# Datou/Datou-gomoku-muzero

Measured on AMD Instinct MI355X. Metric: self-play moves/sec (15x15, 400 sims), higher is better.
Workload: dtype fp16

## Files before the change

### datou-gomoku-muzero_amd/csrc/gmz_conv.hip

```cpp
#include <initializer_list>
#include <type_traits>

#include "gmz_common.h"

#include <hip/hip_bf16.h>
#include <hip/hip_fp16.h>

namespace gmz {
namespace {

typedef _Float16 f16x8_t __attribute__((ext_vector_type(8)));
typedef __bf16 b16x8_t __attribute__((ext_vector_type(8)));
typedef float f32x4_t __attribute__((ext_vector_type(4)));
typedef uint16_t u16x4_t __attribute__((ext_vector_type(4)));

#ifndef GMZ_CONV_RD
#define GMZ_CONV_RD 3
#endif
constexpr int CC = 128;
constexpr int CKSTEPS = 36;
constexpr int FRAG_BYTES = 294912;

__device__ __forceinline__ int csigma16(int j) { return j < 8 ? (j ^ 4) : j; }

template <int H>
struct CImg {
  static constexpr int HP = H + 2, PS = 272, RS = HP * PS - 32;
  static constexpr int BYTES = ((HP - 1) * RS + HP * PS + 255) / 256 * 256;
  static constexpr int RUN = (H - 1) * PS + 256;
  static constexpr int RUN_DMA = (RUN + 1023) / 1024;
};

template <typename T> struct Mfma;
template <> struct Mfma<__half> {
  typedef f16x8_t V;
  static __device__ __forceinline__ f32x4_t run(V a, V b, f32x4_t c) {
    return __builtin_amdgcn_mfma_f32_16x16x32_f16(a, b, c, 0, 0, 0);
  }
  static __device__ __forceinline__ uint16_t bits(float f) { return __builtin_bit_cast(uint16_t, (_Float16)f); }
  static __device__ __forceinline__ float value(uint16_t u) { return (float)__builtin_bit_cast(_Float16, u); }
};
template <> struct Mfma<__hip_bfloat16> {
  typedef b16x8_t V;
  static __device__ __forceinline__ f32x4_t run(V a, V b, f32x4_t c) {
    return __builtin_amdgcn_mfma_f32_16x16x32_bf16(a, b, c, 0, 0, 0);
  }
  static __device__ __forceinline__ uint16_t bits(float f) { return __builtin_bit_cast(uint16_t, (__bf16)f); }
  static __device__ __forceinline__ float value(uint16_t u) { return __uint_as_float(((uint32_t)u) << 16); }
};

__device__ __forceinline__ int chunk_of(int ks, int g) { return 2 * ks + ((g & 1) * 8 + (g >> 1)); }

template <typename T>
__global__ void __launch_bounds__(256) k_pack_conv(const float *__restrict__ w, long s0, long s1, long s2, long s3,
                                                   int transpose, uint16_t *__restrict__ out) {
  const int i = blockIdx.x * 256 + threadIdx.x;
  if (i >= CKSTEPS * 8 * 64) return;
  const int l = i & 63, nt = (i >> 6) & 7, st = i >> 9, t = st >> 2, ks = st & 3;
  const int n = nt * 16 + (l & 15);
  u16x4_t lo, hi;
#pragma unroll
  for (int j = 0; j < 8; ++j) {
    const int c = chunk_of(ks, l >> 4) * 8 + j;
    const int o = transpose ? c : n, ci = transpose ? n : c, tt = transpose ? 8 - t : t;
    const float v = w[o * s0 + ci * s1 + (tt / 3) * s2 + (tt % 3) * s3];
    const uint16_t b = Mfma<T>::bits(v);
    if (j < 4) lo[j] = b;
    else hi[j - 4] = b;
  }
  uint4 r;
  r.x = (uint32_t)lo[0] | ((uint32_t)lo[1] << 16);
  r.y = (uint32_t)lo[2] | ((uint32_t)lo[3] << 16);
  r.z = (uint32_t)hi[0] | ((uint32_t)hi[1] << 16);
  r.w = (uint32_t)hi[2] | ((uint32_t)hi[3] << 16);
  *(uint4 *)(out + (size_t)i * 8) = r;
}

struct PackJob {
  const float *w;
  long long s0, s1, s2, s3;
  uint16_t *out;
  int transpose, pad;
};

template <typename T>
__global__ void __launch_bounds__(256) k_pack_many(const PackJob *__restrict__ jobs) {
  const PackJob j = jobs[blockIdx.y];
  const int i = blockIdx.x * 256 + threadIdx.x;
  if (i >= CKSTEPS * 8 * 64) return;
  const int l = i & 63, nt = (i >> 6) & 7, st = i >> 9, t = st >> 2, ks = st & 3;
  const int n = nt * 16 + (l & 15);
  u16x4_t lo, hi;
#pragma unroll
  for (int e = 0; e < 8; ++e) {
    const int c = chunk_of(ks, l >> 4) * 8 + e;
    const int o = j.transpose ? c : n, ci = j.transpose ? n : c, tt = j.transpose ? 8 - t : t;
    const uint16_t b = Mfma<T>::bits(j.w[o * j.s0 + ci * j.s1 + (tt / 3) * j.s2 + (tt % 3) * j.s3]);
    if (e < 4) lo[e] = b;
    else hi[e - 4] = b;
  }
  uint4 r;
  r.x = (uint32_t)lo[0] | ((uint32_t)lo[1] << 16);
  r.y = (uint32_t)lo[2] | ((uint32_t)lo[3] << 16);
  r.z = (uint32_t)hi[0] | ((uint32_t)hi[1] << 16);
  r.w = (uint32_t)hi[2] | ((uint32_t)hi[3] << 16);
  *(uint4 *)(j.out + (size_t)i * 8) = r;
}

struct BnBwd {
  const uint16_t *x, *y;
  const float *save;
  int relu;
};

struct ActStamp {
  const int32_t *action;
  const float *table;
};

struct BnApply {
  const uint16_t *z, *res;
  const float *gamma, *beta, *save;
  uint16_t *out;
  int relu;
};

template <int... Hs> struct SizeList {};
using ConvSizes = SizeList<6, 9, 15, 19>;

#ifndef GMZ_CONV_PG19
#define GMZ_CONV_PG19 2
#endif
template <int H> struct ConvCfg { static constexpr int PG = 2, WG_PER_CU = 2; static constexpr bool AB = H == 9 || H == 15; };
template <> struct ConvCfg<19> { static constexpr int PG = GMZ_CONV_PG19, WG_PER_CU = 1; static constexpr bool AB = false; };

template <int H, typename T, int PG, bool BWD = false, bool PB = false, bool BNA = false>
__global__ void __launch_bounds__(128 * PG, ConvCfg<H>::WG_PER_CU) k_conv3(const uint16_t *__restrict__ x, const uint16_t *__restrict__ wpk,
                                                  uint16_t *__restrict__ y, int N, const uint8_t *__restrict__ mask,
                                                  double *__restrict__ stats, const uint16_t *__restrict__ addend,
                                                  BnBwd bn, ActStamp as, BnApply ba) {
  using I = CImg<H>;
  using M = Mfma<T>;
  typedef typename M::V V;
  constexpr int A = H * H, NPT = (A + 15) / 16;
  constexpr int NTW = 2, PTW = (NPT + PG - 1) / PG, RD = GMZ_CONV_RD, NW = 2 * PG, NTHR = 64 * NW;
  constexpr int PS = I::PS, RS = I::RS;
  static_assert(CKSTEPS % RD == 0, "ring slots repeat per item");
  constexpr bool REMAP = false;
  constexpr bool LAST_ONE = !REMAP && NPT == PG * (PTW - 1) + 1;
  constexpr unsigned LAST_TAPS = LAST_ONE ? live_taps(H, (NPT - 1) * 16, A) : 0x1ffu;
  static_assert(LAST_TAPS & 1u, "tap 0 of the last tile starts its accumulation");
  __shared__ __attribute__((aligned(16))) uint8_t img[I::BYTES];
  static_assert(I::BYTES >= PG * 64 * 2 * 4, "stats scratch fits in the image");
  static_assert(!PB || !BWD, "per-board statistics: forward sums");
  static_assert(!BNA || (!BWD && !PB), "BatchNorm-apply prologue: the forward with per-workgroup statistics");
  static_assert(NTHR % 16 == 0, "BNA: a thread's chunk of every cell it stages is tid & 15");
  __shared__ float pbred[PB ? PG * 64 * 2 : 1];

  const int tid = threadIdx.x, w = tid >> 6, lane = tid & 63;
  const int nq = w & 1, pg = w >> 1;
  const int g4 = lane >> 4;
  const int cg = (g4 & 1) * 8 + (g4 >> 1);
  const int half0 = (blockIdx.x >> 3) & 1;
  const int b0 = (int)((blockIdx.x >> 4) * 8 + (blockIdx.x & 7));
  const int bstride = (int)(gridDim.x >> 1);
  const int ntile0 = half0 * 4 + nq * NTW;

  {
    constexpr int HP = I::HP, NBORDER = 2 * HP + 2 * H;
    for (int i = tid; i < NBORDER * 16; i += NTHR) {
      const int k = i >> 4, r = k - 2 * HP;
      const int yy = k < HP ? 0 : k < 2 * HP ? HP - 1 : 1 + (r >> 1);
      const int xx = k < HP ? k : k < 2 * HP ? k - HP : (r & 1) * (HP - 1);
      ((uint4 *)(img + yy * RS + xx * PS))[i & 15] = make_uint4(0, 0, 0, 0);
    }
  }

  auto tile_p = [&](int pt) {
    if constexpr (REMAP) {
      const int p = pt < NPT ? remap15(pt, csigma16(lane & 15)) : -1;
      return p < 0 ? A : p;
    }
    const int p = pt * 16 + csigma16(lane & 15);
    return (pt < NPT && p < A) ? p : A;
  };
  int pos[PTW];
#pragma unroll
  for (int i = 0; i < PTW; ++i) {
    const int pt = pg + PG * i, p = tile_p(pt);
    const int pad = REMAP ? 16 * ((remap15_key0(pt) + csigma16(lane & 15)) & 15)
                          : ((A - 1) / H) * RS + ((A - 1) % H) * PS;
    pos[i] = p < A ? (p / H) * RS + (p % H) * PS : ~pad;
  }
  const __amdgpu_buffer_rsrc_t wrsrc = __builtin_amdgcn_make_buffer_rsrc((void *)wpk, (short)0, FRAG_BYTES, 0x00020000);
  const int wvoff = ntile0 * 1024 + lane * 16;
  V ar[RD][NTW];
  auto loadA = [&](int slot, int st) {
    const int soff = (st < CKSTEPS ? st : st - CKSTEPS) * 8192;
#pragma unroll
    for (int nt = 0; nt < NTW; ++nt)
      ar[slot][nt] = __builtin_bit_cast(V, __builtin_amdgcn_raw_buffer_load_b128(wrsrc, wvoff + nt * 1024, soff, 0));
  };
#pragma unroll
  for (int k = 0; k < RD - 1; ++k) loadA(k, k);
  __syncthreads();
  float s1[NTW][4], s2[NTW][4];
#pragma unroll
  for (int nt = 0; nt < NTW; ++nt)
#pragma unroll
    for (int e = 0; e < 4; ++e) s1[nt][e] = s2[nt][e] = 0.f;
  int nvalid = 0;

  auto dma = [&](int bd) {
    const uint8_t *src = (const uint8_t *)(x + (size_t)bd * A * CC);
    for (int j = w; j < H * I::RUN_DMA; j += NW) {
      const int yy = j / I::RUN_DMA, piece = j % I::RUN_DMA;
      const int o = piece * 1024 + lane * 16;
      const int xx = o / PS, ch = (o % PS) >> 4;
      if (o < I::RUN && ch < 16)
        __builtin_amdgcn_global_load_lds((const void *)(src + (yy * H + xx) * 256 + ch * 16),
                                         (__attribute__((address_space(3))) void *)(img + (yy + 1) * RS + PS + piece * 1024),
                                         16, 0, 0);
    }
  };
  auto bn_stage = [&](int bd) {
    int t = tid;
    asm volatile("" : "+v"(t));
    const int bch = t & 15;
    float bmu[8], bsc[8], bsh[8];
#pragma unroll
    for (int j = 0; j < 8; ++j) {
      const int c = bch * 8 + j;
      bmu[j] = ba.save[c];
      bsc[j] = ba.gamma[c] * ba.save[CC + c];
      bsh[j] = ba.beta[c];
    }
    constexpr int NCH = A * 16, NI = (NCH + NTHR - 1) / NTHR, U = 8;
    const size_t base = (size_t)bd * NCH;
    const uint4 *zs = (const uint4 *)ba.z + base;
    const uint4 *rs = ba.res ? (const uint4 *)ba.res + base : nullptr;
    uint4 *os = (uint4 *)ba.out + base;
    const bool mine = (bch >> 3) == half0;
    const uint32_t nz = M::bits(-0.f) * 0x10001u;
    const float lo = ba.relu ? 0.f : -__builtin_inff();
#pragma unroll
    for (int i0 = 0; i0 < NI; i0 += U) {
      uint4 zv[U], rv[U];
#pragma unroll
      for (int u = 0; u < U; ++u) {
        const int i = t + (i0 + u) * NTHR;
        rv[u] = make_uint4(nz, nz, nz, nz);
        if (i0 + u < NI && i < NCH) {
          zv[u] = zs[i];
          if (rs) rv[u] = rs[i];
        }
      }
#pragma unroll
      for (int u = 0; u < U; ++u) {
        const int i = t + (i0 + u) * NTHR;
        if (!(i0 + u < NI && i < NCH)) continue;
        const uint32_t *zw = (const uint32_t *)&zv[u], *rw = (const uint32_t *)&rv[u];
        uint32_t ow[4];
#pragma unroll
        for (int h = 0; h < 4; ++h) {
          uint32_t packed = 0;
#pragma unroll
          for (int e = 0; e < 2; ++e) {
            const int j = 2 * h + e;
            float v = (M::value((uint16_t)(zw[h] >> (16 * e))) - bmu[j]) * bsc[j] + bsh[j];
            v += M::value((uint16_t)(rw[h] >> (16 * e)));
            v = fmaxf(v, lo);
            packed |= (uint32_t)M::bits(v) << (16 * e);
          }
          ow[h] = packed;
        }
        const uint4 o = make_uint4(ow[0], ow[1], ow[2], ow[3]);
        const int p = i >> 4;
        ((uint4 *)(img + (p / H + 1) * RS + (p % H + 1) * PS))[bch] = o;
        if (mine) os[i] = o;
      }
    }
  };
  int mrow = 1;
  if (mask) {
    const int bj = b0 + lane * bstride;
    mrow = bj < N ? (int)mask[bj] : 0;
  }
  for (int b = b0, j = 0; b < N; b += bstride, ++j) {
    if constexpr (BNA) {
      bn_stage(b);
    } else {
      dma(b);
      asm volatile("s_waitcnt vmcnt(0)" ::: "memory");
    }
    __syncthreads();
    const bool counted = stats && (!mask || (j < WAVE ? __builtin_amdgcn_readlane(mrow, j) != 0 : mask[b] != 0));
    nvalid += counted;

    f32x4_t acc[NTW][PTW];
    int bb[PTW];
#pragma unroll
    for (int i = 0; i < PTW; ++i) bb[i] = (pos[i] < 0 ? ~pos[i] : pos[i]) + cg * 16;
    auto kloop = [&](auto ntl_c) {
      constexpr int NTL = decltype(ntl_c)::value;
      V bf[2][NTL];
      constexpr int PGK = NTL == PTW ? 0 : 1;
      auto taps = [&](int i) -> unsigned {
        if constexpr (REMAP) return remap15_taps(PGK + PG * i);
        return (LAST_ONE && NTL == PTW && i == NTL - 1) ? LAST_TAPS : 0x1ffu;
      };
      auto live = [&](int i, int st) { return ((taps(i) >> (st >> 2)) & 1u) != 0; };
      auto first = [&](int i) { return 4 * __builtin_ctz(taps(i)); };
      auto readB = [&](int buf, int st) {
        const int tap = st >> 2, ks = st & 3;
        const int off = (tap / 3) * RS + (tap % 3) * PS + ks * 32;
#pragma unroll
        for (int i = 0; i < NTL; ++i)
          if (live(i, st)) bf[buf][i] = *(const V *)(img + bb[i] + off);
      };
      readB(0, 0);
#pragma unroll
      for (int st = 0; st < CKSTEPS; ++st) {
        loadA((st + RD - 1) % RD, st + RD - 1);
        if (st + 1 < CKSTEPS) readB((st + 1) & 1, st + 1);
        __builtin_amdgcn_sched_barrier(0);
#pragma unroll
        for (int i = 0; i < NTL; ++i)
          if (live(i, st))
#pragma unroll
            for (int nt = 0; nt < NTW; ++nt)
              acc[nt][i] = M::run(ar[st % RD][nt], bf[st & 1][i], st == first(i) ? f32x4_t{0.f, 0.f, 0.f, 0.f} : acc[nt][i]);
        if (st + 1 < CKSTEPS) __builtin_amdgcn_sched_barrier(0);
      }
#pragma unroll
      for (int i = NTL; i < PTW; ++i)
#pragma unroll
        for (int nt = 0; nt < NTW; ++nt) acc[nt][i] = f32x4_t{0.f, 0.f, 0.f, 0.f};
    };
    if constexpr (PTW * PG == NPT) kloop(std::integral_constant<int, PTW>{});
    else if (pg + PG * (PTW - 1) < NPT) kloop(std::integral_constant<int, PTW>{});
    else kloop(std::integral_constant<int, PTW - 1>{});

    uint16_t *dst = y + (size_t)b * A * CC;
    int say = -100, sax = -100;
    if (as.action) {
      const int av = as.action[b];
      say = av / H;
      sax = av - say * H;
    }
    const uint16_t *add = addend ? addend + (size_t)b * A * CC : nullptr;
    float mu[NTW][4], isd[NTW][4];
    if constexpr (BWD) {
#pragma unroll
      for (int nt = 0; nt < NTW; ++nt)
#pragma unroll
        for (int e = 0; e < 4; ++e) {
          const int c = (ntile0 + nt) * 16 + g4 * 4 + e;
          mu[nt][e] = bn.save[c];
          isd[nt][e] = bn.save[CC + c];
        }
    }
#pragma unroll
    for (int i = 0; i < PTW; ++i) {
      const int p = tile_p(pg + PG * i);
      if (p >= A) continue;
#pragma unroll
      for (int nt = 0; nt < NTW; ++nt) {
        const int n0 = (ntile0 + nt) * 16 + g4 * 4;
        u16x4_t o;
        {
          const int ddy = say - p / H + 1, ddx = sax - p % H + 1;
          if (ddy >= 0 && ddy <= 2 && ddx >= 0 && ddx <= 2) {
            const float *tb = as.table + (ddy * 3 + ddx) * CC + n0;
#pragma unroll
            for (int e = 0; e < 4; ++e) acc[nt][i][e] += tb[e];
          }
        }
        if (add) {
          const u16x4_t ad = *(const u16x4_t *)(add + (size_t)p * CC + n0);
#pragma unroll
          for (int e = 0; e < 4; ++e) o[e] = M::bits(acc[nt][i][e] + M::value(ad[e]));
        } else {
#pragma unroll
          for (int e = 0; e < 4; ++e) o[e] = M::bits(acc[nt][i][e]);
        }
        *(u16x4_t *)(dst + (size_t)p * CC + n0) = o;
        if (counted) {
          if constexpr (BWD) {
            const size_t k = ((size_t)b * A + p) * CC + n0;
            const u16x4_t xv = *(const u16x4_t *)(bn.x + k), yv = *(const u16x4_t *)(bn.y + k);
#pragma unroll
            for (int e = 0; e < 4; ++e) {
              float g = M::value(o[e]);
              if (bn.relu && !(M::value(yv[e]) > 0.f)) g = 0.f;
              s1[nt][e] += g;
              s2[nt][e] = fmaf(g, (M::value(xv[e]) - mu[nt][e]) * isd[nt][e], s2[nt][e]);
            }
          } else {
#pragma unroll
            for (int e = 0; e < 4; ++e) {
              const float v = M::value(o[e]);
              s1[nt][e] += v;
              s2[nt][e] = fmaf(v, v, s2[nt][e]);
            }
          }
        }
      }
    }
    if constexpr (PB) {
      if (stats) {
#pragma unroll
        for (int nt = 0; nt < NTW; ++nt)
#pragma unroll
          for (int e = 0; e < 4; ++e)
#pragma unroll
            for (int o = 1; o < 16; o <<= 1) {
              s1[nt][e] += __shfl_xor(s1[nt][e], o, 64);
              s2[nt][e] += __shfl_xor(s2[nt][e], o, 64);
            }
        if ((lane & 15) == 0) {
#pragma unroll
          for (int nt = 0; nt < NTW; ++nt)
#pragma unroll
            for (int e = 0; e < 4; ++e) {
              const int cl = (nq * NTW + nt) * 16 + g4 * 4 + e;
              pbred[(pg * 64 + cl) * 2] = s1[nt][e];
              pbred[(pg * 64 + cl) * 2 + 1] = s2[nt][e];
            }
        }
#pragma unroll
        for (int nt = 0; nt < NTW; ++nt)
#pragma unroll
          for (int e = 0; e < 4; ++e) s1[nt][e] = s2[nt][e] = 0.f;
        __syncthreads();
        if (tid < 64) {
          double a = 0.0, q = 0.0;
#pragma unroll
          for (int g = 0; g < PG; ++g) {
            a += (double)pbred[(g * 64 + tid) * 2];
            q += (double)pbred[(g * 64 + tid) * 2 + 1];
          }
          double *out = stats + ((size_t)(half0 * 64 + tid) * N + b) * 3;
          out[0] = a;
          out[1] = q;
          out[2] = counted ? (double)A : 0.0;
// ... 140 lines not shown
        arl[slot][nt] = __builtin_bit_cast(
            V, __builtin_amdgcn_raw_buffer_load_b128(wrsrc, wvoff + nt * 1024, FRAG_BYTES + st * 8192, 0));
    }
  };
#pragma unroll
  for (int k = 0; k < RD - 1; ++k) loadA(k, k);

  auto stage = [&](int bd, auto lo_c) {
    constexpr bool LO = decltype(lo_c)::value;
    int t = tid;
    asm volatile("" : "+v"(t));
    const int bch = t & 15;
    constexpr int NCH = A * 16, NI = (NCH + NTHR - 1) / NTHR, U = 4;
    const float4 *src = (const float4 *)(x + (size_t)bd * A * CC);
#pragma unroll
    for (int i0 = 0; i0 < NI; i0 += U) {
      float4 va[U], vb[U];
#pragma unroll
      for (int u = 0; u < U; ++u) {
        const int i = t + (i0 + u) * NTHR;
        if (i0 + u < NI && i < NCH) {
          va[u] = src[2 * i];
          vb[u] = src[2 * i + 1];
        }
      }
#pragma unroll
      for (int u = 0; u < U; ++u) {
        const int i = t + (i0 + u) * NTHR;
        if (!(i0 + u < NI && i < NCH)) continue;
        const float f[8] = {va[u].x, va[u].y, va[u].z, va[u].w, vb[u].x, vb[u].y, vb[u].z, vb[u].w};
        uint32_t ow[4];
#pragma unroll
        for (int h = 0; h < 4; ++h) {
          const uint16_t e0 = LO ? split_lo(f[2 * h]) : split_hi(f[2 * h]);
          const uint16_t e1 = LO ? split_lo(f[2 * h + 1]) : split_hi(f[2 * h + 1]);
          ow[h] = (uint32_t)e0 | ((uint32_t)e1 << 16);
        }
        const int p = i >> 4;
        ((uint4 *)(img + (p / H + 1) * RS + (p % H + 1) * PS))[bch] = make_uint4(ow[0], ow[1], ow[2], ow[3]);
      }
    }
  };

  for (int b = b0; b < N; b += bstride) {
    f32x4_t am[NTW][PTW], ac[NTW][PTW];
#pragma unroll
    for (int nt = 0; nt < NTW; ++nt)
#pragma unroll
      for (int i = 0; i < PTW; ++i) am[nt][i] = ac[nt][i] = f32x4_t{0.f, 0.f, 0.f, 0.f};
    auto kloop = [&](auto ntl_c, auto pass_c) {
      constexpr int NTL = decltype(ntl_c)::value, PASS = decltype(pass_c)::value;
      V bf[NTL];
      auto live = [&](int i, int st) {
        const unsigned taps = (LAST_ONE && NTL == PTW && i == NTL - 1) ? LAST_TAPS : 0x1ffu;
        return ((taps >> (st >> 2)) & 1u) != 0;
      };
      auto readB = [&](int i, int st) {
        const int tap = st >> 2, ks = st & 3;
        bf[i] = *(const V *)(img + bb[i] + (tap / 3) * RS + (tap % 3) * PS + ks * 32);
      };
#pragma unroll
      for (int i = 0; i < NTL; ++i) readB(i, 0);
#pragma unroll
      for (int st = 0; st < CKSTEPS; ++st) {
        constexpr int S0 = PASS * CKSTEPS;
        loadA((S0 + st + RD - 1) % RD, S0 + st + RD - 1);
#pragma unroll
        for (int i = 0; i < NTL; ++i) {
          if (live(i, st)) {
#pragma unroll
            for (int nt = 0; nt < NTW; ++nt) {
              if constexpr (PASS == 0) {
                am[nt][i] = M::run(arh[(S0 + st) % RD][nt], bf[i], am[nt][i]);
                ac[nt][i] = M::run(arl[(S0 + st) % RD][nt], bf[i], ac[nt][i]);
              } else {
                ac[nt][i] = M::run(arh[(S0 + st) % RD][nt], bf[i], ac[nt][i]);
              }
            }
          }
          if (st + 1 < CKSTEPS && live(i, st + 1)) readB(i, st + 1);
          __builtin_amdgcn_sched_barrier(0);
        }
      }
    };
    auto pass = [&](auto pass_c) {
      if constexpr (PTW * PG == NPT) kloop(std::integral_constant<int, PTW>{}, pass_c);
      else if (pg + PG * (PTW - 1) < NPT) kloop(std::integral_constant<int, PTW>{}, pass_c);
      else kloop(std::integral_constant<int, PTW - 1>{}, pass_c);
    };
    stage(b, std::false_type{});
    __syncthreads();
    pass(std::integral_constant<int, 0>{});
    __syncthreads();
    stage(b, std::true_type{});
    __syncthreads();
    pass(std::integral_constant<int, 1>{});

    int ln = lane;
    asm volatile("" : "+v"(ln));
    const int eg4 = ln >> 4, ecol = csigma16(ln & 15);
    float *dst = y + (size_t)b * A * CC;
    const float *rsd = bn.res ? bn.res + (size_t)b * A * CC : nullptr;
    float mu[NTW][4], sc[NTW][4], sh[NTW][4];
    if (bn.gamma) {
#pragma unroll
      for (int nt = 0; nt < NTW; ++nt)
#pragma unroll
        for (int e = 0; e < 4; ++e) {
          const int c = (ntile0 + nt) * 16 + eg4 * 4 + e;
          mu[nt][e] = bn.mean[c];
          sc[nt][e] = bn.gamma[c] * (1.0f / sqrtf(bn.var[c] + bn.eps));
          sh[nt][e] = bn.beta[c];
        }
    }
#pragma unroll
    for (int i = 0; i < PTW; ++i) {
      const int pt = pg + PG * i, p = pt * 16 + ecol;
      if (pt >= NPT || p >= A) continue;
#pragma unroll
      for (int nt = 0; nt < NTW; ++nt) {
        const int n0 = (ntile0 + nt) * 16 + eg4 * 4;
        f32x4_t o;
#pragma unroll
        for (int e = 0; e < 4; ++e) o[e] = am[nt][i][e] + ac[nt][i][e] * SPLIT_INV;
        if (bn.gamma) {
          f32x4_t r = {0.f, 0.f, 0.f, 0.f};
          if (rsd) r = *(const f32x4_t *)(rsd + (size_t)p * CC + n0);
#pragma unroll
          for (int e = 0; e < 4; ++e) {
            float v = (o[e] - mu[nt][e]) * sc[nt][e] + sh[nt][e];
            if (rsd) v += r[e];
            o[e] = bn.relu ? fmaxf(v, 0.f) : v;
          }
        }
        *(f32x4_t *)(dst + (size_t)p * CC + n0) = o;
      }
    }
    __syncthreads();
  }
}

typedef short s16x4_t __attribute__((ext_vector_type(4)));

template <int H>
struct WgLds {
  static constexpr int A = H * H, RB = 288, HP = H + 2;
  static constexpr int NB = H > 15 ? 2 : 1, BR = (H + NB - 1) / NB;
  static constexpr int BA = BR * H;
  static constexpr int KS = (BA + 31) / 32, NPOS = KS * 32;
  static constexpr int DY_BYTES = NPOS * RB, X_OFF = DY_BYTES, X_BYTES = (NB == 1 ? HP : BR) * HP * RB;
  static constexpr int BYTES = DY_BYTES + X_BYTES;
  static constexpr int NPD = (BA * RB + 1023) / 1024;
  static constexpr int RUN = (H - 1) * RB + 256, RUN_DMA = (RUN + 1023) / 1024;
};

__device__ __forceinline__ s16x4_t tr_read(const uint8_t *lds_base, int off) {
  return __builtin_amdgcn_ds_read_tr16_b64_v4i16((__attribute__((address_space(3))) s16x4_t *)(
      (__attribute__((address_space(3))) uint8_t *)lds_base + off));
}

constexpr int WG_MAX_SEGS = 8;
struct WgSrc {
  const uint16_t *x[WG_MAX_SEGS];
  const uint16_t *dy[WG_MAX_SEGS];
  int nps;
};

template <int H, typename T>
__global__ void __launch_bounds__(512, 1) k_conv3_wgrad(WgSrc src, int N, int nch, float *__restrict__ part) {
  using L = WgLds<H>;
  using M = Mfma<T>;
  typedef typename M::V V;
  constexpr int A = H * H, KS = L::KS, RB = L::RB, HP = L::HP;
  static_assert(L::BYTES <= 163840, "LDS budget");
  __shared__ __attribute__((aligned(16))) uint8_t smem[L::BYTES];
  uint8_t *xt = smem + L::X_OFF;

  const int tid = threadIdx.x, w = tid >> 6, lane = tid & 63;
  const int xcd = blockIdx.x & 7, slot = blockIdx.x >> 3;
  const int ty = slot % 3, chunk = (slot / 3) * 8 + xcd;
  const int wo = w & 3, wc = w >> 2;
  const int g = lane >> 4, q = (lane >> 2) & 3, pp = lane & 3;
  const int ocol = (wo * 32 + 4 * pp) * 2, ccol = (wc * 64 + 4 * pp) * 2;

  auto zero_cell = [&](uint8_t *cellp, int i) { ((uint4 *)cellp)[i & 15] = make_uint4(0, 0, 0, 0); };
  if constexpr (L::NB == 1) {
    constexpr int NTAIL = L::NPOS - A, NBORDER = 2 * HP + 2 * H;
    for (int i = tid; i < (NTAIL + NBORDER) * 16; i += 512) {
      const int k = i >> 4;
      uint8_t *cellp;
      if (k < NTAIL) {
        cellp = smem + (A + k) * RB;
      } else {
        const int kb = k - NTAIL, r = kb - 2 * HP;
        const int yy = kb < HP ? 0 : kb < 2 * HP ? HP - 1 : 1 + (r >> 1);
        const int xx = kb < HP ? kb : kb < 2 * HP ? kb - HP : (r & 1) * (HP - 1);
        cellp = xt + (yy * HP + xx) * RB;
      }
      ((uint4 *)cellp)[i & 15] = make_uint4(0, 0, 0, 0);
    }
  } else {
    constexpr int NTAIL = L::NPOS - L::BA, NBORDER = 2 * L::BR;
    for (int i = tid; i < (NTAIL + NBORDER) * 16; i += 512) {
      const int k = i >> 4, kb = k - NTAIL;
      zero_cell(k < NTAIL ? smem + (L::BA + k) * RB : xt + ((kb >> 1) * HP + (kb & 1) * (HP - 1)) * RB, i);
    }
  }
  __syncthreads();

  f32x4_t acc[3][2][4];
#pragma unroll
  for (int tx = 0; tx < 3; ++tx)
#pragma unroll
    for (int mt = 0; mt < 2; ++mt)
#pragma unroll
      for (int nt = 0; nt < 4; ++nt) acc[tx][mt][nt] = f32x4_t{0.f, 0.f, 0.f, 0.f};

  for (int b = chunk; b < N; b += nch) {
    const int sg = b / src.nps, lb = b - sg * src.nps;
    const uint8_t *sd = (const uint8_t *)(src.dy[sg] + (size_t)lb * A * CC);
    const uint8_t *sx = (const uint8_t *)(src.x[sg] + (size_t)lb * A * CC);
    if constexpr (L::NB == 1) {
      for (int j = w; j < L::NPD + H * L::RUN_DMA; j += 8) {
        if (j < L::NPD) {
          const int o = j * 1024 + lane * 16;
          const int row = o / RB, ch = (o % RB) >> 4;
          if (row < A && ch < 16)
            __builtin_amdgcn_global_load_lds((const void *)(sd + row * 256 + ch * 16),
                                             (__attribute__((address_space(3))) void *)(smem + j * 1024), 16, 0, 0);
        } else {
          const int jj = j - L::NPD, yy = jj / L::RUN_DMA, piece = jj % L::RUN_DMA;
          const int o = piece * 1024 + lane * 16;
          const int xx = o / RB, ch = (o % RB) >> 4;
          if (o < L::RUN && ch < 16)
            __builtin_amdgcn_global_load_lds((const void *)(sx + (yy * H + xx) * 256 + ch * 16),
                                             (__attribute__((address_space(3))) void *)(xt + ((yy + 1) * HP + 1) * RB + piece * 1024),
                                             16, 0, 0);
        }
      }
      asm volatile("s_waitcnt vmcnt(0)" ::: "memory");
      __syncthreads();
#pragma unroll 2
      for (int ks = 0; ks < KS; ++ks) {
        const int p0 = ks * 32 + 4 * g + q, p1 = p0 + 16;
        const int c0 = p0 < A ? p0 : A - 1, c1 = p1 < A ? p1 : A - 1;
        const int xb0 = ((c0 / H + ty) * HP + c0 % H) * RB + ccol, xb1 = ((c1 / H + ty) * HP + c1 % H) * RB + ccol;
        const int ab0 = p0 * RB + ocol, ab1 = p1 * RB + ocol;
        V af[2];
#pragma unroll
        for (int mt = 0; mt < 2; ++mt) {
          const s16x4_t lo = tr_read(smem, ab0 + mt * 32), hi = tr_read(smem, ab1 + mt * 32);
          af[mt] = __builtin_bit_cast(V, __builtin_shufflevector(lo, hi, 0, 1, 2, 3, 4, 5, 6, 7));
        }
#pragma unroll
        for (int tx = 0; tx < 3; ++tx) {
#pragma unroll
          for (int nt = 0; nt < 4; ++nt) {
            const s16x4_t lo = tr_read(xt, xb0 + tx * RB + nt * 32), hi = tr_read(xt, xb1 + tx * RB + nt * 32);
            const V bf = __builtin_bit_cast(V, __builtin_shufflevector(lo, hi, 0, 1, 2, 3, 4, 5, 6, 7));
#pragma unroll
            for (int mt = 0; mt < 2; ++mt) acc[tx][mt][nt] = M::run(af[mt], bf, acc[tx][mt][nt]);
          }
        }
      }
      __syncthreads();
    } else {
      for (int bd = 0; bd < L::NB; ++bd) {
        const int r0 = bd * L::BR, nrows = H - r0 < L::BR ? H - r0 : L::BR, npos = nrows * H;
        const int xr0 = r0 + ty - 1;
        const int zrow = xr0 < 0 ? 0 : xr0 + nrows > H ? nrows - 1 : -1;
        const int ntail = L::BA - npos, nz = ntail + (zrow >= 0 ? H : 0);
        for (int i = tid; i < nz * 16; i += 512) {
          const int k = i >> 4;
          zero_cell(k < ntail ? smem + (npos + k) * RB : xt + (zrow * HP + 1 + (k - ntail)) * RB, i);
        }
        for (int j = w; j < L::NPD + nrows * L::RUN_DMA; j += 8) {
          if (j < L::NPD) {
            const int o = j * 1024 + lane * 16;
            const int row = o / RB, ch = (o % RB) >> 4;
            if (row < npos && ch < 16)
              __builtin_amdgcn_global_load_lds((const void *)(sd + (r0 * H + row) * 256 + ch * 16),
                                               (__attribute__((address_space(3))) void *)(smem + j * 1024), 16, 0, 0);
          } else {
            const int jj = j - L::NPD, yy = jj / L::RUN_DMA, piece = jj % L::RUN_DMA;
            const int o = piece * 1024 + lane * 16;
            const int xx = o / RB, ch = (o % RB) >> 4;
            if (yy != zrow && o < L::RUN && ch < 16)
              __builtin_amdgcn_global_load_lds((const void *)(sx + ((xr0 + yy) * H + xx) * 256 + ch * 16),
                                               (__attribute__((address_space(3))) void *)(xt + (yy * HP + 1) * RB + piece * 1024),
                                               16, 0, 0);
          }
        }
        asm volatile("s_waitcnt vmcnt(0)" ::: "memory");
        __syncthreads();
#pragma unroll 2
        for (int ks = 0; ks < KS; ++ks) {
          const int p0 = ks * 32 + 4 * g + q, p1 = p0 + 16;
          const int c0 = p0 < npos ? p0 : npos - 1, c1 = p1 < npos ? p1 : npos - 1;
          const int xb0 = (c0 / H * HP + c0 % H) * RB + ccol, xb1 = (c1 / H * HP + c1 % H) * RB + ccol;
          const int ab0 = p0 * RB + ocol, ab1 = p1 * RB + ocol;
          V af[2];
#pragma unroll
          for (int mt = 0; mt < 2; ++mt) {
            const s16x4_t lo = tr_read(smem, ab0 + mt * 32), hi = tr_read(smem, ab1 + mt * 32);
            af[mt] = __builtin_bit_cast(V, __builtin_shufflevector(lo, hi, 0, 1, 2, 3, 4, 5, 6, 7));
          }
#pragma unroll
          for (int tx = 0; tx < 3; ++tx) {
#pragma unroll
            for (int nt = 0; nt < 4; ++nt) {
              const s16x4_t lo = tr_read(xt, xb0 + tx * RB + nt * 32), hi = tr_read(xt, xb1 + tx * RB + nt * 32);
              const V bf = __builtin_bit_cast(V, __builtin_shufflevector(lo, hi, 0, 1, 2, 3, 4, 5, 6, 7));
#pragma unroll
              for (int mt = 0; mt < 2; ++mt) acc[tx][mt][nt] = M::run(af[mt], bf, acc[tx][mt][nt]);
            }
          }
        }
        __syncthreads();
      }
    }
  }
  float *pc = part + (size_t)chunk * 9 * CC * CC;
#pragma unroll
  for (int tx = 0; tx < 3; ++tx)
#pragma unroll
    for (int mt = 0; mt < 2; ++mt)
#pragma unroll
      for (int nt = 0; nt < 4; ++nt)
#pragma unroll
        for (int e = 0; e < 4; ++e) {
          const int o = wo * 32 + 16 * mt + 4 * g + e, c = wc * 64 + 16 * nt + (lane & 15);
          pc[((size_t)(ty * 3 + tx) * CC + o) * CC + c] = acc[tx][mt][nt][e];
        }
}

__global__ void __launch_bounds__(256) k_conv3_wgrad_reduce(const float *__restrict__ part, int nch, float *dw, long s0,
                                                            long s1, long s2, long s3, int accumulate) {
  const int i = blockIdx.x * 256 + threadIdx.x;
  if (i >= 9 * CC * CC) return;
  const int c = i % CC, o = (i / CC) % CC, t = i / (CC * CC);
  constexpr size_t STR = 9 * CC * CC;
  float s[8] = {0.f, 0.f, 0.f, 0.f, 0.f, 0.f, 0.f, 0.f};
  int k = 0;
  for (; k + 8 <= nch; k += 8) {
#pragma unroll
    for (int u = 0; u < 8; ++u) s[u] += part[(size_t)(k + u) * STR + i];
  }
  for (; k < nch; ++k) s[0] += part[(size_t)k * STR + i];
  const float tot = ((s[0] + s[1]) + (s[2] + s[3])) + ((s[4] + s[5]) + (s[6] + s[7]));
  float *d = dw + o * s0 + c * s1 + (t / 3) * s2 + (t % 3) * s3;
  *d = accumulate ? *d + tot : tot;
}

static int cu_count_conv() {
  static int n = 0;
  if (!n) {
    int dev = 0;
    (void)hipGetDevice(&dev);
    hipDeviceProp_t p;
    n = hipGetDeviceProperties(&p, dev) == hipSuccess ? p.multiProcessorCount : 256;
  }
  return n;
}

int conv3_grid(int N) {
  const long items = (2L * N + 15) / 16 * 16, cap = 2L * 2 * cu_count_conv() / 16 * 16;
  return (int)(items < cap ? items : cap);
}

int conv3_stats_slots(int N, bool per_board = false) { return per_board ? N : conv3_grid(N) / 2; }
static int check_slots(const char *fn, const double *stats, int stats_slots, int N, bool per_board) {
  if (!stats) return 0;
  const int need = conv3_stats_slots(N, per_board);
  if (stats_slots != need)
    return fail(std::string(fn) + ": statistics buffer of " + std::to_string(stats_slots) + " slots, this launch writes " +
// ... 292 lines not shown
```

Baseline: 12630.

## Stage BN-apply input via LDS DMA and vectorize BN math in conv kernel

```diff
diff --git a/datou-gomoku-muzero_amd/csrc/gmz_conv.hip b/datou-gomoku-muzero_amd/csrc/gmz_conv.hip
--- a/datou-gomoku-muzero_amd/csrc/gmz_conv.hip
+++ b/datou-gomoku-muzero_amd/csrc/gmz_conv.hip
@@ -12,10 +12,16 @@
 typedef _Float16 f16x8_t __attribute__((ext_vector_type(8)));
 typedef __bf16 b16x8_t __attribute__((ext_vector_type(8)));
 typedef float f32x4_t __attribute__((ext_vector_type(4)));
+typedef float f32x2_t __attribute__((ext_vector_type(2)));
+typedef _Float16 f16x2_t __attribute__((ext_vector_type(2)));
+typedef __bf16 b16x2_t __attribute__((ext_vector_type(2)));
 typedef uint16_t u16x4_t __attribute__((ext_vector_type(4)));
 
 #ifndef GMZ_CONV_RD
 #define GMZ_CONV_RD 3
+#endif
+#ifndef GMZ_BNA_STAGE
+#define GMZ_BNA_STAGE 2
 #endif
 constexpr int CC = 128;
 constexpr int CKSTEPS = 36;
@@ -39,6 +45,12 @@
   }
   static __device__ __forceinline__ uint16_t bits(float f) { return __builtin_bit_cast(uint16_t, (_Float16)f); }
   static __device__ __forceinline__ float value(uint16_t u) { return (float)__builtin_bit_cast(_Float16, u); }
+  static __device__ __forceinline__ f32x2_t value2(uint32_t u) {
+    return __builtin_convertvector(__builtin_bit_cast(f16x2_t, u), f32x2_t);
+  }
+  static __device__ __forceinline__ uint32_t bits2(f32x2_t f) {
+    return __builtin_bit_cast(uint32_t, __builtin_convertvector(f, f16x2_t));
+  }
 };
 template <> struct Mfma<__hip_bfloat16> {
   typedef b16x8_t V;
@@ -47,6 +59,12 @@
   }
   static __device__ __forceinline__ uint16_t bits(float f) { return __builtin_bit_cast(uint16_t, (__bf16)f); }
   static __device__ __forceinline__ float value(uint16_t u) { return __uint_as_float(((uint32_t)u) << 16); }
+  static __device__ __forceinline__ f32x2_t value2(uint32_t u) {
+    return f32x2_t{__uint_as_float(u << 16), __uint_as_float(u & 0xffff0000u)};
+  }
+  static __device__ __forceinline__ uint32_t bits2(f32x2_t f) {
+    return __builtin_bit_cast(uint32_t, __builtin_convertvector(f, b16x2_t));
+  }
 };
 
 __device__ __forceinline__ int chunk_of(int ks, int g) { return 2 * ks + ((g & 1) * 8 + (g >> 1)); }
@@ -211,8 +229,8 @@
     for (int e = 0; e < 4; ++e) s1[nt][e] = s2[nt][e] = 0.f;
   int nvalid = 0;
 
-  auto dma = [&](int bd) {
-    const uint8_t *src = (const uint8_t *)(x + (size_t)bd * A * CC);
+  auto dma = [&](const uint16_t *from, int bd) {
+    const uint8_t *src = (const uint8_t *)(from + (size_t)bd * A * CC);
     for (int j = w; j < H * I::RUN_DMA; j += NW) {
       const int yy = j / I::RUN_DMA, piece = j % I::RUN_DMA;
       const int o = piece * 1024 + lane * 16;
@@ -235,14 +253,86 @@
       bsc[j] = ba.gamma[c] * ba.save[CC + c];
       bsh[j] = ba.beta[c];
     }
-    constexpr int NCH = A * 16, NI = (NCH + NTHR - 1) / NTHR, U = 8;
+    constexpr int NCH = A * 16, NI = (NCH + NTHR - 1) / NTHR, U = (GMZ_BNA_STAGE == 0 || H > 15) ? 8 : NI;
     const size_t base = (size_t)bd * NCH;
-    const uint4 *zs = (const uint4 *)ba.z + base;
     const uint4 *rs = ba.res ? (const uint4 *)ba.res + base : nullptr;
     uint4 *os = (uint4 *)ba.out + base;
     const bool mine = (bch >> 3) == half0;
     const uint32_t nz = M::bits(-0.f) * 0x10001u;
     const float lo = ba.relu ? 0.f : -__builtin_inff();
+    auto apply = [&](const uint4 &zq, const uint4 &rq) {
+      const uint32_t *zw = (const uint32_t *)&zq, *rw = (const uint32_t *)&rq;
+      uint32_t ow[4];
+#pragma unroll
+      for (int h = 0; h < 4; ++h) {
+#if GMZ_BNA_STAGE == 2
+        f32x2_t v = (M::value2(zw[h]) - f32x2_t{bmu[2 * h], bmu[2 * h + 1]}) * f32x2_t{bsc[2 * h], bsc[2 * h + 1]} +
+                    f32x2_t{bsh[2 * h], bsh[2 * h + 1]};
+        v += M::value2(rw[h]);
+        v.x = fmaxf(v.x, lo);
+        v.y = fmaxf(v.y, lo);
+        ow[h] = M::bits2(v);
+#else
+        uint32_t packed = 0;
+#pragma unroll
+        for (int e = 0; e < 2; ++e) {
+          const int j = 2 * h + e;
+          float v = (M::value((uint16_t)(zw[h] >> (16 * e))) - bmu[j]) * bsc[j] + bsh[j];
+          v += M::value((uint16_t)(rw[h] >> (16 * e)));
+          v = fmaxf(v, lo);
+          packed |= (uint32_t)M::bits(v) << (16 * e);
+        }
+        ow[h] = packed;
+#endif
+      }
+      return make_uint4(ow[0], ow[1], ow[2], ow[3]);
+    };
+#if GMZ_BNA_STAGE == 2
+    dma(ba.z, bd);
+    auto has = [&](int k) { return (k + 1) * NTHR <= NCH || (k < NI && t + k * NTHR < NCH); };
+    constexpr int UL = U < 8 ? U : 8;
+    uint4 zv[UL], rv[U];
+    auto load_res = [&](int i0) {
+#pragma unroll
+      for (int u = 0; u < U; ++u) rv[u] = make_uint4(nz, nz, nz, nz);
+      if (rs) {
+#pragma unroll
+        for (int u = 0; u < U; ++u)
+          if (has(i0 + u)) rv[u] = rs[t + (i0 + u) * NTHR];
+      }
+    };
+    load_res(0);
+    constexpr int DY = (NTHR / 16) / H, DX = (NTHR / 16) % H;
+    int cx = (t >> 4) % H, ca = ((t >> 4) / H + 1) * RS + (cx + 1) * PS + bch * 16;
+    asm volatile("s_waitcnt vmcnt(0)" ::: "memory");
+    __syncthreads();
+#pragma unroll
+    for (int i0 = 0; i0 < NI; i0 += U) {
+      if (i0 > 0) load_res(i0);
+#pragma unroll
+      for (int u0 = 0; u0 < U; u0 += UL) {
+        int at[UL];
+#pragma unroll
+        for (int u = 0; u < UL; ++u) {
+          at[u] = ca;
+          if (u0 + u < U && has(i0 + u0 + u)) zv[u] = *(const uint4 *)(img + ca);
+          const bool wrap = cx + DX >= H;
+          cx += DX - (wrap ? H : 0);
+          ca += DY * RS + DX * PS + (wrap ? RS - H * PS : 0);
+        }
+#pragma unroll
+        for (int u = 0; u < UL; ++u)
+          if (u0 + u < U && has(i0 + u0 + u)) *(uint4 *)(img + at[u]) = zv[u] = apply(zv[u], rv[u0 + u]);
+        if (mine) {
+#pragma unroll
+          for (int u = 0; u < UL; ++u)
+            if (u0 + u < U && has(i0 + u0 + u)) os[t + (i0 + u0 + u) * NTHR] = zv[u];
+        }
+      }
+    }
+#else
+    auto chunk_at = [&](int i) { return (uint4 *)(img + ((i >> 4) / H + 1) * RS + ((i >> 4) % H + 1) * PS) + bch; };
+    const uint4 *zs = (const uint4 *)ba.z + base;
 #pragma unroll
     for (int i0 = 0; i0 < NI; i0 += U) {
       uint4 zv[U], rv[U];
@@ -259,27 +349,12 @@
       for (int u = 0; u < U; ++u) {
         const int i = t + (i0 + u) * NTHR;
         if (!(i0 + u < NI && i < NCH)) continue;
-        const uint32_t *zw = (const uint32_t *)&zv[u], *rw = (const uint32_t *)&rv[u];
-        uint32_t ow[4];
-#pragma unroll
-        for (int h = 0; h < 4; ++h) {
-          uint32_t packed = 0;
-#pragma unroll
-          for (int e = 0; e < 2; ++e) {
-            const int j = 2 * h + e;
-            float v = (M::value((uint16_t)(zw[h] >> (16 * e))) - bmu[j]) * bsc[j] + bsh[j];
-            v += M::value((uint16_t)(rw[h] >> (16 * e)));
-            v = fmaxf(v, lo);
-            packed |= (uint32_t)M::bits(v) << (16 * e);
-          }
-          ow[h] = packed;
-        }
-        const uint4 o = make_uint4(ow[0], ow[1], ow[2], ow[3]);
-        const int p = i >> 4;
-        ((uint4 *)(img + (p / H + 1) * RS + (p % H + 1) * PS))[bch] = o;
+        const uint4 o = apply(zv[u], rv[u]);
+        *chunk_at(i) = o;
         if (mine) os[i] = o;
       }
     }
+#endif
   };
   int mrow = 1;
   if (mask) {
@@ -290,7 +365,7 @@
     if constexpr (BNA) {
       bn_stage(b);
     } else {
-      dma(b);
+      dma(x, b);
       asm volatile("s_waitcnt vmcnt(0)" ::: "memory");
     }
     __syncthreads();
```

Result: no change. 12640 (median of 2 runs) (+0.1%).

## Double-buffer 15x15 conv weight-gradient LDS loads across two half-sample units

Applied to the files above, without the earlier changes.

```diff
diff --git a/datou-gomoku-muzero_amd/csrc/gmz_conv.hip b/datou-gomoku-muzero_amd/csrc/gmz_conv.hip
--- a/datou-gomoku-muzero_amd/csrc/gmz_conv.hip
+++ b/datou-gomoku-muzero_amd/csrc/gmz_conv.hip
@@ -737,6 +737,17 @@
   static constexpr int BYTES = DY_BYTES + X_BYTES;
   static constexpr int NPD = (BA * RB + 1023) / 1024;
   static constexpr int RUN = (H - 1) * RB + 256, RUN_DMA = (RUN + 1023) / 1024;
+  static constexpr bool PIPE = H == 15;
+  static constexpr int UKS = KS / 2, UPOS = UKS * 32, R1 = UPOS / H, XR0 = (UPOS - 1) / H + 1, XR1 = H - R1;
+  static constexpr int B0 = (UPOS + XR0 * HP) * RB, B1 = (UPOS + XR1 * HP) * RB;
+  static constexpr int LDS_BYTES = PIPE ? B0 : BYTES, LDS1_BYTES = PIPE ? B1 : 1;
+};
+
+template <int H, int UNIT>
+struct WgUnit {
+  using L = WgLds<H>;
+  static constexpr int U = UNIT, NROW = U ? L::A - L::UPOS : L::UPOS, NPD = (NROW * L::RB + 1023) / 1024;
+  static constexpr int NP = NPD + (U ? L::XR1 : L::XR0) * L::RUN_DMA, NI = (NP + 7) / 8;
 };
 
 __device__ __forceinline__ s16x4_t tr_read(const uint8_t *lds_base, int off) {
@@ -757,8 +768,9 @@
   using M = Mfma<T>;
   typedef typename M::V V;
   constexpr int A = H * H, KS = L::KS, RB = L::RB, HP = L::HP;
-  static_assert(L::BYTES <= 163840, "LDS budget");
-  __shared__ __attribute__((aligned(16))) uint8_t smem[L::BYTES];
+  static_assert(L::LDS_BYTES + L::LDS1_BYTES <= 163840, "LDS budget");
+  __shared__ __attribute__((aligned(16))) uint8_t smem[L::LDS_BYTES];
+  __shared__ __attribute__((aligned(16))) uint8_t smem1[L::LDS1_BYTES];
   uint8_t *xt = smem + L::X_OFF;
 
   const int tid = threadIdx.x, w = tid >> 6, lane = tid & 63;
@@ -769,7 +781,20 @@
   const int ocol = (wo * 32 + 4 * pp) * 2, ccol = (wc * 64 + 4 * pp) * 2;
 
   auto zero_cell = [&](uint8_t *cellp, int i) { ((uint4 *)cellp)[i & 15] = make_uint4(0, 0, 0, 0); };
-  if constexpr (L::NB == 1) {
+  if constexpr (L::PIPE) {
+    constexpr int NTAIL = L::NPOS - A, NB0 = 2 * L::XR0, NB1 = 2 * L::XR1;
+    uint8_t *x0 = smem + L::UPOS * RB, *d1 = smem1, *x1 = d1 + L::UPOS * RB;
+    const int nz = NTAIL + NB0 + NB1 + (ty != 1 ? H : 0);
+    for (int i = tid; i < nz * 16; i += 512) {
+      int k = i >> 4;
+      uint8_t *cellp;
+      if (k < NTAIL) cellp = d1 + (A - L::UPOS + k) * RB;
+      else if ((k -= NTAIL) < NB0) cellp = x0 + ((k >> 1) * HP + (k & 1) * (HP - 1)) * RB;
+      else if ((k -= NB0) < NB1) cellp = x1 + ((k >> 1) * HP + (k & 1) * (HP - 1)) * RB;
+      else cellp = (ty == 0 ? x0 : x1 + (L::XR1 - 1) * HP * RB) + (1 + k - NB1) * RB;
+      zero_cell(cellp, i);
+    }
+  } else if constexpr (L::NB == 1) {
     constexpr int NTAIL = L::NPOS - A, NBORDER = 2 * HP + 2 * H;
     for (int i = tid; i < (NTAIL + NBORDER) * 16; i += 512) {
       const int k = i >> 4;
@@ -801,11 +826,88 @@
 #pragma unroll
       for (int nt = 0; nt < 4; ++nt) acc[tx][mt][nt] = f32x4_t{0.f, 0.f, 0.f, 0.f};
 
+  const int wu = __builtin_amdgcn_readfirstlane(w);
+  auto piece_src = [&](auto uc, int j) {
+    using P = WgUnit<H, decltype(uc)::value>;
+    if (j < P::NPD) {
+      const int o = j * 1024 + lane * 16;
+      const int row = o / RB, ch = (o % RB) >> 4;
+      return row < P::NROW && ch < 16 ? (P::U * L::UPOS + row) * 256 + ch * 16 : -1;
+    }
+    const int jj = j - P::NPD, yy = jj / L::RUN_DMA, piece = jj % L::RUN_DMA;
+    const int o = piece * 1024 + lane * 16;
+    const int xx = o / RB, ch = (o % RB) >> 4, br = P::U * L::R1 + ty - 1 + yy;
+    return j < P::NP && br >= 0 && br < H && o < L::RUN && ch < 16 ? (br * H + xx) * 256 + ch * 16 : -1;
+  };
+  int so0[WgUnit<H, 0>::NI], so1[WgUnit<H, 1>::NI];
+  if constexpr (L::PIPE) {
+#pragma unroll
+    for (int i = 0; i < WgUnit<H, 0>::NI; ++i) so0[i] = piece_src(std::integral_constant<int, 0>{}, wu + 8 * i);
+#pragma unroll
+    for (int i = 0; i < WgUnit<H, 1>::NI; ++i) so1[i] = piece_src(std::integral_constant<int, 1>{}, wu + 8 * i);
+  }
+  auto unit_dma = [&](auto uc, const auto &so, int b) {
+    using P = WgUnit<H, decltype(uc)::value>;
+    uint8_t *bd = P::U ? smem1 : smem;
+    const int sg = b / src.nps, lb = b - sg * src.nps;
+    const uint8_t *sd = (const uint8_t *)(src.dy[sg] + (size_t)lb * A * CC);
+    const uint8_t *sx = (const uint8_t *)(src.x[sg] + (size_t)lb * A * CC);
+#pragma unroll
+    for (int i = 0; i < P::NI; ++i) {
+      const int j = wu + 8 * i, jj = j - P::NPD;
+      if (j >= P::NP) break;
+      const int dst = j < P::NPD ? j * 1024 : (L::UPOS + jj / L::RUN_DMA * HP + 1) * RB + jj % L::RUN_DMA * 1024;
+      if (so[i] >= 0)
+        __builtin_amdgcn_global_load_lds((const void *)((j < P::NPD ? sd : sx) + (unsigned)so[i]),
+                                         (__attribute__((address_space(3))) void *)(bd + dst), 16, 0, 0);
+    }
+  };
+  auto unit_ksteps = [&](auto uc) {
+    constexpr int U = decltype(uc)::value;
+    const uint8_t *bd = U ? smem1 : smem, *bx = bd + L::UPOS * RB;
+#pragma unroll 2
+    for (int ks = 0; ks < L::UKS; ++ks) {
+      const int l0 = ks * 32 + 4 * g + q, l1 = l0 + 16, p0 = U * L::UPOS + l0, p1 = p0 + 16;
+      const int c0 = p0 < A ? p0 : A - 1, c1 = p1 < A ? p1 : A - 1;
+      const int xb0 = ((c0 / H - U * L::R1) * HP + c0 % H) * RB + ccol;
+      const int xb1 = ((c1 / H - U * L::R1) * HP + c1 % H) * RB + ccol;
+      const int ab0 = l0 * RB + ocol, ab1 = l1 * RB + ocol;
+      V af[2];
+#pragma unroll
+      for (int mt = 0; mt < 2; ++mt) {
+        const s16x4_t lo = tr_read(bd, ab0 + mt * 32), hi = tr_read(bd, ab1 + mt * 32);
+        af[mt] = __builtin_bit_cast(V, __builtin_shufflevector(lo, hi, 0, 1, 2, 3, 4, 5, 6, 7));
+      }
+#pragma unroll
+      for (int tx = 0; tx < 3; ++tx) {
+#pragma unroll
+        for (int nt = 0; nt < 4; ++nt) {
+          const s16x4_t lo = tr_read(bx, xb0 + tx * RB + nt * 32), hi = tr_read(bx, xb1 + tx * RB + nt * 32);
+          const V bf = __builtin_bit_cast(V, __builtin_shufflevector(lo, hi, 0, 1, 2, 3, 4, 5, 6, 7));
+#pragma unroll
+          for (int mt = 0; mt < 2; ++mt) acc[tx][mt][nt] = M::run(af[mt], bf, acc[tx][mt][nt]);
+        }
+      }
+    }
+  };
+  if constexpr (L::PIPE) {
+    if (chunk < N) unit_dma(std::integral_constant<int, 0>{}, so0, chunk);
+  }
+
   for (int b = chunk; b < N; b += nch) {
     const int sg = b / src.nps, lb = b - sg * src.nps;
     const uint8_t *sd = (const uint8_t *)(src.dy[sg] + (size_t)lb * A * CC);
     const uint8_t *sx = (const uint8_t *)(src.x[sg] + (size_t)lb * A * CC);
-    if constexpr (L::NB == 1) {
+    if constexpr (L::PIPE) {
+      asm volatile("s_waitcnt vmcnt(0)" ::: "memory");
+      __syncthreads();
+      unit_dma(std::integral_constant<int, 1>{}, so1, b);
+      unit_ksteps(std::integral_constant<int, 0>{});
+      asm volatile("s_waitcnt vmcnt(0)" ::: "memory");
+      __syncthreads();
+      if (b + nch < N) unit_dma(std::integral_constant<int, 0>{}, so0, b + nch);
+      unit_ksteps(std::integral_constant<int, 1>{});
+    } else if constexpr (L::NB == 1) {
       for (int j = w; j < L::NPD + H * L::RUN_DMA; j += 8) {
         if (j < L::NPD) {
           const int o = j * 1024 + lane * 16;
```

Result: no change. 12290 before, 12280 after (-0.1%).
